# timothydmorton/isochrones

Measured on AMD Instinct MI355X. Metric: lnpost evals/sec over MIST grid (10^6-sample batch), higher is better.
Workload: dtype f64

## Files before the change

### isochrones_amd/csrc/fast/lnpost_wave.h

```cpp
#pragma once

#ifndef ISO_LANE_BC_MAX_BANDS
#define ISO_LANE_BC_MAX_BANDS 1
#endif
constexpr int LANE_BC_MAX_BANDS = ISO_LANE_BC_MAX_BANDS;
template <int KIND, int NS, int NB, bool ASTERO = false, bool MASKED = false, bool TILED = false, bool STDP = false,
          int LANE = 0>
__device__ __forceinline__ double lnpost_wave(const FastArgs& A, const double* lds, const CoopLds& L, bool active,
                                              const DevModel& M, const DevModel& MP, const double* __restrict__ p, bool want_parts,
                                              double& lnp_out, double& lnl_out)
{
    const double q1 = p[NS], feh_par = p[NS + 1], dist = p[NS + 2], AV = p[NS + 3];

    const double x0 = (KIND == ISO_KIND_TRACK) ? p[2] : q1;
    const double x1 = (KIND == ISO_KIND_TRACK) ? p[0] : feh_par;
    const bool ok01 = bool(active & !(x0 != x0) & !(x1 != x1) & !lds_oob(lds, A.m0, x0) & !lds_oob(lds, A.m1, x1));
    int i0, i1;
    W3 w;
    w.t2 = 0.0;
    lds_bracket2(lds, A.m0, A.m1, x0, x1, i0, i1, w.t0, w.t1);
    constexpr int K_MASS = STDP ? ISO_PRIOR_CHABRIER : -1, K_AGE = STDP ? ISO_PRIOR_FLATLOG : -1, K_FEH = STDP ? ISO_PRIOR_FEH : -1,
                  K_DIST = STDP ? ISO_PRIOR_POWERLAW : -1, K_AV = STDP ? ISO_PRIOR_FLAT : -1;
    constexpr bool OVERLAP = (LANE & 4) != 0 && (LANE & 1) == 0;
    constexpr bool THREE = (LANE & 8) != 0 || ISO_COOP_STAR3 != 0;
    double ld = 0.0, t_first = 0.0, t_feh = 0.0, t_dist = 0.0, t_av = 0.0;
    auto table_free_priors = [&]() {
        ld = fast_log(dist);
        t_first = (KIND == ISO_KIND_TRACK) ? ln_pdf<false, K_MASS>(MP.prior_mass, p[0], 0.0) : ln_pdf<false, K_AGE>(MP.prior_age, q1, 0.0);
        t_feh = ln_pdf<false, K_FEH>(MP.prior_feh, feh_par, 0.0);
        t_dist = ln_pdf<true, K_DIST>(M.prior_distance, dist, ld);
        t_av = ln_pdf<false, K_AV>(MP.prior_AV, AV, 0.0);
    };
    double star[NS][6];
    double astero[2] = {0.0, 0.0};
    constexpr bool SPREAD = (LANE & (16 | 32)) != 0;
    static_assert(!SPREAD || (((LANE & 16) ? NS == 2 : NS == 3) && (LANE & 48) != 48 && KIND == ISO_KIND_ISO && !TILED && !ASTERO && (LANE & 1) == 0),
                  "one star per lane: binaries (bit 4) / triples (bit 5) on the isochrone grid, cooperative model gather");
    const int my_star = !SPREAD ? 0 : (NS == 2 ? (L.lane >> 5) : ((L.lane >> 4) < 2 ? (L.lane >> 4) : 2));
    const bool my_row = !SPREAD || NS == 2 || (L.lane >> 4) < 3;
    if constexpr (SPREAD) {
        double eep = p[0];
#pragma unroll
        for (int s = 1; s < NS; ++s) eep = my_star == s ? p[s] : eep;
        const bool ok = bool(ok01 & my_row & !(eep != eep) & !eep_oob(A, eep));
        int i2;
        eep_bracket(A, lds, eep, i2, w.t2);
        const uint32_t cell = cell3(A, i0, i1, i2);
        double mine[6];
        if constexpr (OVERLAP) coop_star<true, decltype(table_free_priors)&, true, THREE>(A, L, ok, cell, w, mine, table_free_priors);
        else coop_star<false, NoWorkBetween, true, THREE>(A, L, ok, cell, w, mine);
#pragma unroll
        for (int q = 0; q < 6; ++q) {
            double each[NS];
            stars_f64<NS>(mine[q], each);
#pragma unroll
            for (int s = 0; s < NS; ++s) star[s][q] = each[s];
        }
    }
#pragma unroll
    for (int s = 0; s < (SPREAD ? 0 : NS); ++s) {
        const double eep = (KIND == ISO_KIND_TRACK) ? p[1] : p[s];
        const bool ok = bool(ok01 & !(eep != eep) & !eep_oob(A, eep));
        int i2;
        eep_bracket(A, lds, eep, i2, w.t2);
        {
            uint32_t cell = cell3(A, i0, i1, i2);
            ISO_STAMP(2, cell);
            if constexpr (LANE & 1) lane_star(A, ok, cell, w, star[s]);
            else if constexpr (OVERLAP) {
                if (s == 0) coop_star<true, decltype(table_free_priors)&, false, THREE>(A, L, ok, cell, w, star[s], table_free_priors);
                else coop_star<false, NoWorkBetween, false, THREE>(A, L, ok, cell, w, star[s]);
            } else coop_star<false, NoWorkBetween, false, THREE>(A, L, ok, cell, w, star[s]);
            ISO_STAMP(3, star[s][0]);
            if (ASTERO && s == 0) {
                if constexpr (LANE & 1) lane_pair(A.astq, ok && M.has_numax, cell, w, astero);
                else coop_pair(A.astq, L, ok && M.has_numax, cell, w, astero);
            }
        }
    }

    if constexpr (!OVERLAP) table_free_priors();
    double lnp = 0.0;
    bool rejected = false;
    if (NS == 2) rejected = p[1] > p[0];
    if (NS == 3) rejected = !(p[0] > p[1]) && (p[1] > p[2]);
    if (KIND == ISO_KIND_TRACK) lnp += t_first;
#pragma unroll
    for (int s = 0; s < NS; ++s) {
        const double eep = (KIND == ISO_KIND_TRACK) ? p[1] : p[s];
        lnp += (KIND == ISO_KIND_TRACK) ? eep_term<K_AGE>(MP, MP.prior_age, eep, star[s][4], star[s][5])
                                        : eep_term<K_MASS>(MP, MP.prior_mass, eep, star[s][4], star[s][5]);
    }
    if (KIND == ISO_KIND_ISO) lnp += t_first;
    lnp += t_feh;
    lnp += t_dist;
    lnp += t_av;
    if (rejected) lnp = -f_inf();
    ISO_STAMP(4, lnp);
    const bool prior_ok = active && isfinite(lnp);
    const bool go = active && (prior_ok || want_parts);
    lnp_out = lnp;
    lnl_out = f_nan();

    double lnl = 0.0;
#pragma unroll
    for (int q = 0; q < 3; ++q) {
        if constexpr (STDP) {
            const double val = M.spec_val[q], g0 = M.spec_g0[q], hinv = M.spec_hinv[q];
            const double r = val - star[0][q];
            const double term = g0 - r * r * hinv;
            lnl += (val == val) ? term : 0.0;
        } else {
            const double val = M.spec_val[q];
            if (val == val) {
                const double r = val - star[0][q];
                lnl += M.spec_g0[q] - r * r * M.spec_hinv[q];
            }
        }
    }
    const double dm = fma(ld, 5.0 * kInvLn10, -5.0);
    constexpr bool PLX_EARLY = (LANE & 4) != 0;
    double plx_term = 0.0;
    if constexpr (PLX_EARLY) {
        if (M.has_parallax) {
            const double r = M.plx_val - 1000.0 / dist;
            plx_term = M.plx_g0 - r * r * M.plx_hinv;
        }
    }
    if constexpr (TILED) {
        static_assert(NB > 0, "a band tile has at least one band");
        const int nbt = A.nb_total;
        const bool okA = bool(go & !(AV != AV) & !lds_oob(lds, A.b3, AV));
        bool okb[NS];
        uint32_t cellb[NS];
        W4 wb[NS];
    #pragma unroll
        for (int s = 0; s < NS; ++s) {
            const double T = star[s][0], g = star[s][1], f = star[s][2];
            okb[s] = bool(okA & !(T != T) & !(g != g) & !(f != f) & !lds_oob(lds, A.b0, T) & !lds_oob(lds, A.b1, g) &
                          !lds_oob(lds, A.b2, f));
            int j0, j1, j2, j3;
            lds_bracket4(lds, A.b0, A.b1, A.b2, A.b3, T, g, f, AV, j0, j1, j2, j3, wb[s].t0, wb[s].t1, wb[s].t2, wb[s].t3);
            cellb[s] = cell4(A, j0, j1, j2, j3);
        }
        for (int b0 = 0; b0 < nbt; b0 += NB) {
            double tot[NB], rel[NS > 1 ? NB : 1];
    #pragma unroll
            for (int s = 0; s < NS; ++s) {
                double bc[NB];
                coop_bc_tile<NB>(A, L, okb[s], cellb[s], wb[s], nbt, b0, bc);
    #pragma unroll
                for (int b = 0; b < NB; ++b) {
                    const double mag = star[s][3] + dm - bc[b];
                    if (NS == 1) {
                        tot[b] = mag;
                    } else if (s == 0) {
                        const bool far = fabs(mag) > 700.0;
                        tot[b] = far ? 0.0 : mag;
                        rel[b] = 1.0;
                        if (__ballot(far)) rel[b] = far ? exp10(-0.4 * mag) : 1.0;
                    } else {
                        rel[b] += exp10(-0.4 * (mag - tot[b]));
                    }
                }
            }
    #pragma unroll
            for (int b = 0; b < NB; ++b) {
                const int band = min(b0 + b, nbt - 1);
                const double mag = (NS == 1) ? tot[b] : fma(-2.5, fast_log10(rel[b]), tot[b]);
                const double mv = M.mag_val[band];
                const double r = mv - mag;
                if (b0 + b < nbt && (!MASKED || mv == mv)) lnl += M.mag_g0[band] - r * r * M.mag_hinv[band];
            }
        }
    } else if constexpr (SPREAD && NB > 0) {
        double tot[NB], rel[NB];
        const bool okA = bool(go & !(AV != AV) & !lds_oob(lds, A.b3, AV));
        double bcm[NB];
        {
            double T = star[0][0], g = star[0][1], f = star[0][2];
#pragma unroll
            for (int s = 1; s < NS; ++s) {
                T = my_star == s ? star[s][0] : T;
                g = my_star == s ? star[s][1] : g;
                f = my_star == s ? star[s][2] : f;
            }
            const bool ok = bool(okA & my_row & !(T != T) & !(g != g) & !(f != f) & !lds_oob(lds, A.b0, T) &
                                 !lds_oob(lds, A.b1, g) & !lds_oob(lds, A.b2, f));
            int j0, j1, j2, j3;
            W4 w4v;
            lds_bracket4(lds, A.b0, A.b1, A.b2, A.b3, T, g, f, AV, j0, j1, j2, j3, w4v.t0, w4v.t1, w4v.t2, w4v.t3);
            const uint32_t cell = cell4(A, j0, j1, j2, j3);
            if constexpr ((LANE & 2) != 0 && NB <= LANE_BC_MAX_BANDS) lane_bc<NB>(A, ok, cell, w4v, bcm);
            else coop_bc<NB, true>(A, L, ok, cell, w4v, bcm);
        }
    #pragma unroll
        for (int b = 0; b < NB; ++b) {
            double bcs[NS];
            stars_f64<NS>(bcm[b], bcs);
            {
                const double mag = star[0][3] + dm - bcs[0];
                const bool far = fabs(mag) > 700.0;
                tot[b] = far ? 0.0 : mag;
                rel[b] = 1.0;
                if (__ballot(far)) rel[b] = far ? exp10(-0.4 * mag) : 1.0;
            }
    #pragma unroll
            for (int s = 1; s < NS; ++s) {
                const double mag = star[s][3] + dm - bcs[s];
                rel[b] += exp10(-0.4 * (mag - tot[b]));
            }
        }
    #pragma unroll
        for (int b = 0; b < NB; ++b) {
            const double mag = fma(-2.5, fast_log10(rel[b]), tot[b]);
            if constexpr (STDP) {
                const double mv = M.mag_val[b], g0 = M.mag_g0[b], hinv = M.mag_hinv[b];
                const double r = mv - mag;
                const double term = g0 - r * r * hinv;
                lnl += (!MASKED || mv == mv) ? term : 0.0;
            } else {
                const double r = M.mag_val[b] - mag;
                if (!MASKED || M.mag_val[b] == M.mag_val[b]) lnl += M.mag_g0[b] - r * r * M.mag_hinv[b];
            }
        }
    } else if constexpr (NB > 0) {
        double tot[NB], rel[NS > 1 ? NB : 1];
        const bool okA = bool(go & !(AV != AV) & !lds_oob(lds, A.b3, AV));
    #pragma unroll
        for (int s = 0; s < NS; ++s) {
            const double T = star[s][0], g = star[s][1], f = star[s][2];
            const bool ok = bool(okA & !(T != T) & !(g != g) & !(f != f) & !lds_oob(lds, A.b0, T) &
                                 !lds_oob(lds, A.b1, g) & !lds_oob(lds, A.b2, f));
            double bc[NB];
            int j0, j1, j2, j3;
            W4 w4v;
            lds_bracket4(lds, A.b0, A.b1, A.b2, A.b3, T, g, f, AV, j0, j1, j2, j3, w4v.t0, w4v.t1, w4v.t2, w4v.t3);
            {
                uint32_t cell = cell4(A, j0, j1, j2, j3);
                ISO_STAMP(5, cell);
                if constexpr ((LANE & 2) != 0 && NB <= LANE_BC_MAX_BANDS) lane_bc<NB>(A, ok, cell, w4v, bc);
                else coop_bc<NB>(A, L, ok, cell, w4v, bc);
                ISO_STAMP(6, bc[0]);
            }
    #pragma unroll
            for (int b = 0; b < NB; ++b) {
                const double mag = star[s][3] + dm - bc[b];
                if (NS == 1) {
                    tot[b] = mag;
                } else if (s == 0) {
                    const bool far = fabs(mag) > 700.0;
                    tot[b] = far ? 0.0 : mag;
                    rel[b] = 1.0;
                    if (__ballot(far)) rel[b] = far ? exp10(-0.4 * mag) : 1.0;
                } else {
                    rel[b] += exp10(-0.4 * (mag - tot[b]));
                }
            }
        }
    #pragma unroll
        for (int b = 0; b < NB; ++b) {
            const double mag = (NS == 1) ? tot[b] : fma(-2.5, fast_log10(rel[b]), tot[b]);
            if constexpr (STDP) {
                const double mv = M.mag_val[b], g0 = M.mag_g0[b], hinv = M.mag_hinv[b];
                const double r = mv - mag;
                const double term = g0 - r * r * hinv;
                lnl += (!MASKED || mv == mv) ? term : 0.0;
            } else {
                const double r = M.mag_val[b] - mag;
                if (!MASKED || M.mag_val[b] == M.mag_val[b]) lnl += M.mag_g0[b] - r * r * M.mag_hinv[b];
            }
        }
    }
    if (M.has_parallax) {
        if constexpr (PLX_EARLY) {
            lnl += plx_term;
        } else {
            const double r = M.plx_val - 1000.0 / dist;
            lnl += M.plx_g0 - r * r * M.plx_hinv;
        }
    }
    if (ASTERO && M.has_numax) {
        const double r = M.numax_val - astero[0];
        lnl += M.numax_g0 - r * r * M.numax_hinv;
        if (M.has_dnu) {
            const double r2 = M.dnu_val - astero[1];
            lnl += M.dnu_g0 - r2 * r2 * M.dnu_hinv;
        }
    }
    ISO_STAMP(7, lnl);
    lnl_out = go ? lnl : f_nan();
    return prior_ok ? lnp + lnl : -f_inf();
}

template <int KIND, int NS, int NB, bool ASTERO = false, bool MASKED = false, bool TILED = false, bool STDP = false,
          int LANE = 0>
__device__ __forceinline__ double lnpost_wave(const FastArgs& A, const double* lds, const CoopLds& L, bool active,
                                              const DevModel& M, const double* __restrict__ p, bool want_parts,
                                              double& lnp_out, double& lnl_out)
{
    return lnpost_wave<KIND, NS, NB, ASTERO, MASKED, TILED, STDP, LANE>(A, lds, L, active, M, M, p, want_parts, lnp_out, lnl_out);
}

template <int NB>
__device__ __forceinline__ CoopLds coop_lds(double* lds, int axes_len)
{
    constexpr int REQ_STRIDE = slot_stride(NB);
    const int base = (axes_len + 1) & ~1;
    const int wave = threadIdx.x >> 6;
    CoopLds L;
    L.req = lds + base + wave * 64 * REQ_STRIDE;
    L.rsp = L.req;
    L.stride = REQ_STRIDE;
    L.lane = threadIdx.x & 63;
    return L;
}

#ifdef ISO_FAST_WAVES_MULTI
constexpr int fast_min_waves(int ns, int nb) { return (ns == 1 && nb <= 2) ? 6 : (ns == 1 ? 4 : ISO_FAST_WAVES_MULTI); }
#else
constexpr int fast_min_waves(int ns, int nb)
{
    if (ns == 1) return nb <= 2 ? 6 : 4;
    if (ns == 2) return nb >= 9 ? 3 : 4;
    return nb >= 12 ? 2 : (nb >= 8 ? 3 : 4);
}
#endif

constexpr int WIDE_TILE = 8;
constexpr int wide_tile(int ns) { return ns == 1 ? WIDE_TILE : 4; }

template <int KIND, int NS>
__global__ __launch_bounds__(BLOCK, 4) void k_lnpost_wide(const FastArgs A)
{
    extern __shared__ double lds[];
    for (int j = threadIdx.x; j < A.axes_len; j += BLOCK) lds[j] = A.axes_blob[j];
    __syncthreads();
    const CoopLds L = coop_lds<WIDE_TILE>(lds, A.axes_len);
    const int64_t i = (int64_t)blockIdx.x * BLOCK + threadIdx.x;
    const bool active = i < A.n;
    const int64_t ii = active ? i : (A.n - 1);
    const DevModel& M = A.m[0];
    constexpr int NP = NS + 4;
    double p[NP];
    {
        const double* __restrict__ src = A.pars + ii * A.stride_n;
#pragma unroll
        for (int j = 0; j < NP; ++j) p[j] = src[j * A.stride_p];
    }
    double lnp, lnl;
    const double r = lnpost_wave<KIND, NS, wide_tile(NS), false, false, true>(A, lds, L, active, M, p, A.lnlike != nullptr, lnp, lnl);
    if (active) {
        if (A.lnpost) A.lnpost[i] = r;
        if (A.lnprior) A.lnprior[i] = lnp;
        if (A.lnlike) A.lnlike[i] = lnl;
    }
    if (A.done_flag) {
        __threadfence_system();
        __syncthreads();
        if (threadIdx.x == 0) {
            *reinterpret_cast<volatile unsigned long long*>(A.done_flag) = A.done_seq;
            __threadfence_system();
        }
    }
}

template <int KIND, int NS, int NB, bool MULTI, bool ASTERO = false>
__global__ __launch_bounds__(BLOCK, ASTERO ? (fast_min_waves(NS, NB) > 5 ? 5 : fast_min_waves(NS, NB)) : fast_min_waves(NS, NB))
void k_lnpost_fast(const FastArgs A)
{
    extern __shared__ double lds[];
    for (int j = threadIdx.x; j < A.axes_len; j += BLOCK) lds[j] = A.axes_blob[j];
    __syncthreads();
    const CoopLds L = coop_lds<NB>(lds, A.axes_len);
    const int64_t i = (int64_t)blockIdx.x * BLOCK + threadIdx.x;
    const bool active = i < A.n;
    const int64_t ii = active ? i : (A.n - 1);
    const DevModel& M = A.m[MULTI ? A.star_id[ii] : 0];
    constexpr int NP = NS + 4;
    double p[NP];
    {
        const double* __restrict__ src = A.pars + ii * A.stride_n;
#pragma unroll
        for (int j = 0; j < NP; ++j) p[j] = src[j * A.stride_p];
    }
    double lnp, lnl;
    const DevModel& MP = (MULTI && A.shared_priors) ? A.m[0] : M;
    const double r = lnpost_wave<KIND, NS, NB, ASTERO, MULTI>(A, lds, L, active, M, MP, p, A.lnlike != nullptr, lnp, lnl);
    if (active) {
        if (A.lnpost) A.lnpost[i] = r;
        if (A.lnprior) A.lnprior[i] = lnp;
        if (A.lnlike) A.lnlike[i] = lnl;
    }
    if (A.done_flag) {
        __threadfence_system();
        __syncthreads();
        if (threadIdx.x == 0) {
            *reinterpret_cast<volatile unsigned long long*>(A.done_flag) = A.done_seq;
            __threadfence_system();
        }
    }
}
```

### isochrones_amd/csrc/resources.py

```python
from __future__ import annotations

import json
import re
import subprocess

_FIELDS = {
    "TotalSGPRs": "sgpr", "VGPRs": "vgpr", "AGPRs": "agpr", "ScratchSize [bytes/lane]": "scratch",
    "Occupancy [waves/SIMD]": "waves", "SGPRs Spill": "sgpr_spill", "VGPRs Spill": "vgpr_spill",
    "LDS Size [bytes/block]": "lds",
}
_RE = re.compile(r"remark:\s+(Function Name|" + "|".join(re.escape(k) for k in _FIELDS) + r"): (\S+)")


def is_remark_context(line: str) -> bool:
    return bool(re.match(r"^\s*\d*\s*\|", line))


def demangle(names):
    out = subprocess.run(["c++filt"], input="\n".join(names), capture_output=True, text=True).stdout.split("\n")
    short = []
    for d in out[:len(names)]:
        d = d.replace("(anonymous namespace)::", "").replace("iso::fastk::", "").replace("iso::", "")
        d = re.sub(r"^void ", "", d)
        depth, cut = 0, len(d)
        for i, ch in enumerate(d):
            if ch == "<":
                depth += 1
            elif ch == ">":
                depth -= 1
            elif ch == "(" and depth == 0:
                cut = i
                break
        short.append(d[:cut].strip())
    return short


def parse(text: str) -> dict:
    raw, cur = {}, None
    for m in _RE.finditer(text):
        k, v = m.groups()
        if k == "Function Name":
            cur = raw.setdefault(v, {})
        elif cur is not None:
            cur[_FIELDS[k]] = int(v)
    names = list(raw)
    return dict(zip(demangle(names), (raw[n] for n in names)))


def family(name: str) -> str:
    return name.split("<", 1)[0]


SCRATCH_BUDGET = {
    "k_lnpost_fast": 108,
    "k_lnpost_wide": 20,
    "k_catalog_start": 64,
    "k_stretch_half": 252,
    "k_stretch_persist": 388,
    "k_stretch_pair": 200,
    "k_lnpost": 96,
    "k_lnpost_tree": 16,
    "k_chain_quantiles_exact": 40,
    "k_stretch_isotrack": 24,
    "k_mailbox_tree": 96,
    "k_stretch_tree": 24,
}
DEFAULT_SCRATCH = 0
MAX_AGPR = 0


def violations(table: dict, scratch_budget=None, default_scratch=None, max_agpr=None) -> list:
    sb = SCRATCH_BUDGET if scratch_budget is None else scratch_budget
    ds = DEFAULT_SCRATCH if default_scratch is None else default_scratch
    ma = MAX_AGPR if max_agpr is None else max_agpr
    bad = []
    for name, r in sorted(table.items()):
        if r.get("agpr", 0) > ma:
            bad.append("%s: %d AGPRs (limit %d)" % (name, r["agpr"], ma))
        lim = sb.get(family(name), ds)
        if r.get("scratch", 0) > lim:
            bad.append("%s: %d B/lane of scratch (budget of %s: %d)" % (name, r["scratch"], family(name), lim))
    return bad


def summary(table: dict) -> dict:
    fams = {}
    for name, r in table.items():
        f = fams.setdefault(family(name), {"kernels": 0, "max_vgpr": 0, "max_agpr": 0, "max_scratch": 0, "max_sgpr_spill": 0,
                                           "with_scratch": 0, "with_sgpr_spill": 0, "with_agpr": 0})
        f["kernels"] += 1
        f["max_vgpr"] = max(f["max_vgpr"], r.get("vgpr", 0))
        f["max_agpr"] = max(f["max_agpr"], r.get("agpr", 0))
        f["max_scratch"] = max(f["max_scratch"], r.get("scratch", 0))
        f["max_sgpr_spill"] = max(f["max_sgpr_spill"], r.get("sgpr_spill", 0))
        f["with_scratch"] += r.get("scratch", 0) > 0
        f["with_sgpr_spill"] += r.get("sgpr_spill", 0) > 0
        f["with_agpr"] += r.get("agpr", 0) > 0
    return fams


def render(table: dict) -> str:
    lines = ["%d kernels; %d with AGPRs, %d with scratch, %d with SGPR spills"
             % (len(table), sum(r.get("agpr", 0) > 0 for r in table.values()), sum(r.get("scratch", 0) > 0 for r in table.values()),
                sum(r.get("sgpr_spill", 0) > 0 for r in table.values())), "",
             "%-28s %7s %8s %8s %11s %14s %12s %14s" % ("family", "kernels", "max vgpr", "max agpr", "max scratch", "max sgpr spill",
                                                          "with scratch", "with sgpr spill")]
    for f, s in sorted(summary(table).items()):
        lines.append("%-28s %7d %8d %8d %11d %14d %12d %14d" % (f, s["kernels"], s["max_vgpr"], s["max_agpr"], s["max_scratch"],
                                                               s["max_sgpr_spill"], s["with_scratch"], s["with_sgpr_spill"]))
    lines += ["", "%-78s %5s %5s %5s %7s %5s %6s" % ("kernel", "sgpr", "vgpr", "agpr", "scratch", "waves", "sspill")]
    for name, r in sorted(table.items()):
        lines.append("%-78s %5d %5d %5d %7d %5d %6d" % (name[:78], r.get("sgpr", -1), r.get("vgpr", -1), r.get("agpr", -1),
                                                       r.get("scratch", -1), r.get("waves", -1), r.get("sgpr_spill", -1)))
    return "\n".join(lines) + "\n"


if __name__ == "__main__":
    import sys
    t = parse(open(sys.argv[1], errors="replace").read())
    sys.stdout.write(render(t))
    v = violations(t)
    if v:
        sys.stderr.write("\n".join(v) + "\n")
        sys.exit(1)
```

Baseline: 13.67 billion.

## Stash parameters in LDS gather slot and hoist parameter loads before axis staging

For single-star single-band kernels, the feh, distance and AV parameters are parked in unused doubles of the per-lane LDS gather slot and reloaded after the model gather, cutting live VGPRs so the kernel fits under 80 VGPRs without scratch. Parameter and star-id global loads are issued before the axes are staged into LDS, and the staging loop is unrolled four-wide, so the global latencies overlap. The output index is recomputed from the lane id so threadIdx does not stay live. Per-kernel VGPR/scratch limits are added to the resource checker. The cost is extra LDS traffic and some dependence on the compiler's register allocation.

After: 14.25 billion (median of 6 runs). 1.04x the previous value.

```diff
diff --git a/isochrones_amd/csrc/fast/lnpost_wave.h b/isochrones_amd/csrc/fast/lnpost_wave.h
--- a/isochrones_amd/csrc/fast/lnpost_wave.h
+++ b/isochrones_amd/csrc/fast/lnpost_wave.h
@@ -10,7 +10,10 @@
                                               const DevModel& M, const DevModel& MP, const double* __restrict__ p, bool want_parts,
                                               double& lnp_out, double& lnl_out)
 {
-    const double q1 = p[NS], feh_par = p[NS + 1], dist = p[NS + 2], AV = p[NS + 3];
+    constexpr bool STASH = (LANE & 64) != 0;
+    static_assert(!STASH || (NS == 1 && NB <= 6 && !TILED && (LANE & (1 | 16 | 32)) == 0),
+                  "parameters in the gather slot: doubles 6..8 are free up to six bands; cooperative model gather");
+    double q1 = p[NS], feh_par = p[NS + 1], dist = p[NS + 2], AV = p[NS + 3];
 
     const double x0 = (KIND == ISO_KIND_TRACK) ? p[2] : q1;
     const double x1 = (KIND == ISO_KIND_TRACK) ? p[0] : feh_par;
@@ -19,6 +22,12 @@
     W3 w;
     w.t2 = 0.0;
     lds_bracket2(lds, A.m0, A.m1, x0, x1, i0, i1, w.t0, w.t1);
+    double* const stash = L.req + L.lane * L.stride + 6;
+    if constexpr (STASH) {
+        stash[0] = feh_par;
+        stash[1] = dist;
+        stash[2] = AV;
+    }
     constexpr int K_MASS = STDP ? ISO_PRIOR_CHABRIER : -1, K_AGE = STDP ? ISO_PRIOR_FLATLOG : -1, K_FEH = STDP ? ISO_PRIOR_FEH : -1,
                   K_DIST = STDP ? ISO_PRIOR_POWERLAW : -1, K_AV = STDP ? ISO_PRIOR_FLAT : -1;
     constexpr bool OVERLAP = (LANE & 4) != 0 && (LANE & 1) == 0;
@@ -79,6 +88,12 @@
         }
     }
 
+    if constexpr (STASH) {
+        feh_par = stash[0];
+        dist = stash[1];
+        AV = stash[2];
+    }
+
     if constexpr (!OVERLAP) table_free_priors();
     double lnp = 0.0;
     bool rejected = false;
@@ -276,6 +291,7 @@
         if constexpr (PLX_EARLY) {
             lnl += plx_term;
         } else {
+            if constexpr (STASH) dist = stash[1];
             const double r = M.plx_val - 1000.0 / dist;
             lnl += M.plx_g0 - r * r * M.plx_hinv;
         }
@@ -316,6 +332,23 @@
     return L;
 }
 
+__device__ __forceinline__ void stage_axes(double* lds, const FastArgs& A)
+{
+    const int len = A.axes_len;
+    const double* __restrict__ blob = A.axes_blob;
+    for (int j0 = threadIdx.x; j0 < len; j0 += 4 * BLOCK) {
+        int j[4];
+        double v[4];
+#pragma unroll
+        for (int k = 0; k < 4; ++k) {
+            j[k] = min(j0 + k * BLOCK, len - 1);
+            v[k] = blob[j[k]];
+        }
+#pragma unroll
+        for (int k = 0; k < 4; ++k) lds[j[k]] = v[k];
+    }
+}
+
 #ifdef ISO_FAST_WAVES_MULTI
 constexpr int fast_min_waves(int ns, int nb) { return (ns == 1 && nb <= 2) ? 6 : (ns == 1 ? 4 : ISO_FAST_WAVES_MULTI); }
 #else
@@ -334,13 +367,9 @@
 __global__ __launch_bounds__(BLOCK, 4) void k_lnpost_wide(const FastArgs A)
 {
     extern __shared__ double lds[];
-    for (int j = threadIdx.x; j < A.axes_len; j += BLOCK) lds[j] = A.axes_blob[j];
-    __syncthreads();
-    const CoopLds L = coop_lds<WIDE_TILE>(lds, A.axes_len);
     const int64_t i = (int64_t)blockIdx.x * BLOCK + threadIdx.x;
     const bool active = i < A.n;
     const int64_t ii = active ? i : (A.n - 1);
-    const DevModel& M = A.m[0];
     constexpr int NP = NS + 4;
     double p[NP];
     {
@@ -348,6 +377,10 @@
 #pragma unroll
         for (int j = 0; j < NP; ++j) p[j] = src[j * A.stride_p];
     }
+    stage_axes(lds, A);
+    __syncthreads();
+    const CoopLds L = coop_lds<WIDE_TILE>(lds, A.axes_len);
+    const DevModel& M = A.m[0];
     double lnp, lnl;
     const double r = lnpost_wave<KIND, NS, wide_tile(NS), false, false, true>(A, lds, L, active, M, p, A.lnlike != nullptr, lnp, lnl);
     if (active) {
@@ -370,27 +403,34 @@
 void k_lnpost_fast(const FastArgs A)
 {
     extern __shared__ double lds[];
-    for (int j = threadIdx.x; j < A.axes_len; j += BLOCK) lds[j] = A.axes_blob[j];
-    __syncthreads();
-    const CoopLds L = coop_lds<NB>(lds, A.axes_len);
     const int64_t i = (int64_t)blockIdx.x * BLOCK + threadIdx.x;
     const bool active = i < A.n;
     const int64_t ii = active ? i : (A.n - 1);
-    const DevModel& M = A.m[MULTI ? A.star_id[ii] : 0];
     constexpr int NP = NS + 4;
     double p[NP];
+    int star = 0;
     {
         const double* __restrict__ src = A.pars + ii * A.stride_n;
 #pragma unroll
         for (int j = 0; j < NP; ++j) p[j] = src[j * A.stride_p];
-    }
+        if constexpr (MULTI) star = A.star_id[ii];
+    }
+    stage_axes(lds, A);
+    __syncthreads();
+    const CoopLds L = coop_lds<NB>(lds, A.axes_len);
+    const DevModel& M = A.m[star];
     double lnp, lnl;
     const DevModel& MP = (MULTI && A.shared_priors) ? A.m[0] : M;
-    const double r = lnpost_wave<KIND, NS, NB, ASTERO, MULTI>(A, lds, L, active, M, MP, p, A.lnlike != nullptr, lnp, lnl);
-    if (active) {
-        if (A.lnpost) A.lnpost[i] = r;
-        if (A.lnprior) A.lnprior[i] = lnp;
-        if (A.lnlike) A.lnlike[i] = lnl;
+    constexpr bool SLIM = NS == 1 && NB == 1 && !MULTI && !ASTERO;
+    const double r = lnpost_wave<KIND, NS, NB, ASTERO, MULTI, false, false, SLIM ? 64 : 0>(A, lds, L, active, M, MP, p, A.lnlike != nullptr,
+                                                                                         lnp, lnl);
+    int t = L.lane;
+    asm volatile("" : "+v"(t));
+    const int64_t io = (int64_t)blockIdx.x * BLOCK + (__builtin_amdgcn_readfirstlane(threadIdx.x) & ~63) + t;
+    if (io < A.n) {
+        if (A.lnpost) A.lnpost[io] = r;
+        if (A.lnprior) A.lnprior[io] = lnp;
+        if (A.lnlike) A.lnlike[io] = lnl;
     }
     if (A.done_flag) {
         __threadfence_system();
diff --git a/isochrones_amd/csrc/resources.py b/isochrones_amd/csrc/resources.py
--- a/isochrones_amd/csrc/resources.py
+++ b/isochrones_amd/csrc/resources.py
@@ -67,9 +67,14 @@
 }
 DEFAULT_SCRATCH = 0
 MAX_AGPR = 0
+KERNEL_LIMITS = {
+    "k_lnpost_fast<0, 1, 1, false, false>": {"scratch": 0, "vgpr": 80},
+    "k_lnpost_fast<1, 1, 1, false, false>": {"scratch": 0, "vgpr": 80},
+}
 
 
-def violations(table: dict, scratch_budget=None, default_scratch=None, max_agpr=None) -> list:
+def violations(table: dict, scratch_budget=None, default_scratch=None, max_agpr=None, kernel_limits=None) -> list:
+    kl = KERNEL_LIMITS if kernel_limits is None else kernel_limits
     sb = SCRATCH_BUDGET if scratch_budget is None else scratch_budget
     ds = DEFAULT_SCRATCH if default_scratch is None else default_scratch
     ma = MAX_AGPR if max_agpr is None else max_agpr
@@ -80,6 +85,9 @@
         lim = sb.get(family(name), ds)
         if r.get("scratch", 0) > lim:
             bad.append("%s: %d B/lane of scratch (budget of %s: %d)" % (name, r["scratch"], family(name), lim))
+        for field, most in sorted(kl.get(name, {}).items()):
+            if r.get(field, 0) > most:
+                bad.append("%s: %s = %d (this kernel's limit: %d)" % (name, field, r[field], most))
     return bad
 
 
```
